# Celebrandil/CudaSift

Hardware: AMD Instinct MI355X
Metric: 1920x1080 SIFT frames/sec (higher is better)
Workload: dtype f32

## Files before the change

### cudasift_amd/csrc/kernels_points.hip

```cpp
#include "common.hpp"

#define WAVES_PER_BLOCK 4

__device__ __forceinline__ void wave_sync()
{
  __builtin_amdgcn_fence(__ATOMIC_RELEASE, "wavefront");
  __builtin_amdgcn_wave_barrier();
  __builtin_amdgcn_fence(__ATOMIC_ACQUIRE, "wavefront");
}

template <int CTRL, int ROW_MASK>
__device__ __forceinline__ float dpp_f(float v)
{
  return __builtin_bit_cast(float, __builtin_amdgcn_update_dpp(0, __builtin_bit_cast(int, v), CTRL, ROW_MASK, 0xf, false));
}
#define DPP_QUAD_XOR1 0xB1
#define DPP_QUAD_XOR2 0x4E
#define DPP_ROW_HALF_MIRROR 0x141
#define DPP_ROW_MIRROR 0x140
#define DPP_ROW_BCAST15 0x142
#define DPP_ROW_BCAST31 0x143

__device__ __forceinline__ float wave_sum(float v)
{
// ... 827 lines not shown
  const int stride = gridDim.x * WAVES_PER_BLOCK;
  const int tr = lane >> 4, tc = lane & 15;
  auto fetch = [&](const float4 &k, const OctaveInfo &L, float (&T)[4]) {
    const float *img = scratch + (long long)frame * P.frame_stride + L.img_off;
    const bool sane = k.x > -64.0f && k.y > -64.0f && k.x < (float)(L.w + 64) && k.y < (float)(L.h + 64);
#if ORIENT_FETCH_CONST
    const int x0 = (sane ? 0 : 1) - 7, y0 = -7;
#else
    const int x0 = (int)floorf(sane ? k.x : 0.0f) - 7, y0 = (int)floorf(sane ? k.y : 0.0f) - 7;
#endif
    const unsigned col = (unsigned)clampi(x0 + tc, 0, L.w - 1);
#pragma unroll
    for (int q = 0; q < 4; q++)
      T[q] = *reinterpret_cast<const float *>(reinterpret_cast<const char *>(img) +
                                              (__umul24((unsigned)clampi(y0 + tr + 4 * q, 0, L.h - 1), (unsigned)L.p) + col) * 4u);
  };
  int idx = __builtin_amdgcn_readfirstlane(blockIdx.x * WAVES_PER_BLOCK + wave);
  int o, i, o1 = 0, i1 = 0, o2 = 0, i2 = 0;
  bool more = flat_to_octave(fc, P.noct, idx, o, i);
  if (!more) return;
  float4 cur = *reinterpret_cast<const float4 *>(&fdet[(size_t)(o - 1) * max_pts + i]), nxt = cur, nxt2 = cur;
  bool more1 = flat_to_octave(fc, P.noct, idx + stride, o1, i1);
  if (more1) nxt = *reinterpret_cast<const float4 *>(&fdet[(size_t)(o1 - 1) * max_pts + i1]);
  float T[4];
  fetch(cur, P.o[o], T);
  while (more) {
    const OctaveInfo &L = P.o[o];
    const float *img = scratch + (long long)frame * P.frame_stride + L.img_off;
    Detection *d = &fdet[(size_t)(o - 1) * max_pts + i];
    const int co = o;
    const bool sane = cur.x > -64.0f && cur.y > -64.0f && cur.x < (float)(L.w + 64) && cur.y < (float)(L.h + 64);
    const int x0 = (int)floorf(sane ? cur.x : 0.0f) - 7, y0 = (int)floorf(sane ? cur.y : 0.0f) - 7;
#pragma unroll
    for (int q = 0; q < 4; q++) s_tile[wave][lane + 64 * q] = T[q];
    wave_sync();
    if (more1) fetch(nxt, P.o[o1], T);
    const bool more2 = more1 && flat_to_octave(fc, P.noct, idx + 2 * stride, o2, i2);
    if (more2) nxt2 = *reinterpret_cast<const float4 *>(&fdet[(size_t)(o2 - 1) * max_pts + i2]);
    const OrientResult r = sane ? orient_core_tile(img, L.w, L.h, L.p, q8, cur.x, cur.y, cur.z, s_tile[wave], x0, y0,
                                                   s_hist[wave], s_gauss[wave], s_smp[wave], s_tgrid[wave], lane)
                                : orient_core(img, L.w, L.h, L.p, q8, cur.x, cur.y, cur.z, s_hist[wave], s_gauss[wave],
                                              s_smp[wave], s_tgrid[wave], lane);
    if (lane == 0) {
      d->ori1 = r.ori1;
      d->ori2 = r.ori2;
      d->dupslot = r.has2 ? (int)atomicAdd(&cnt[CNT_DUP + co], 1u) : -1;
    }
    idx += stride;
    more = more1; o = o1; i = i1; cur = nxt;
    more1 = more2; o1 = o2; i1 = i2; nxt = nxt2;
  }
}

template <bool UNROLL>
__device__ __forceinline__ void descr_samples_tile(const float *tile, int x0, int y0, bool q8, float px, float py,
                                                   float sina, float cosa, float ssina, float scosa,
                                                   const float *gauss, int lane, float (&vx)[4], float (&vy)[4],
                                                   int (&ang)[4])
{
  const int tx = lane & 15;
  const float fx = tx - 7.5f, gx = gauss[tx];
  const float *porg = tile_origin<PW>(tile, x0, y0);
#pragma unroll
  for (int j = 0; j < 4; j++) { vx[j] = 0.0f; vy[j] = 0.0f; ang[j] = 0; }
  if (UNROLL) {
#pragma unroll
    for (int j = 0; j < 4; j++) {
      const int y = (lane >> 4) + 4 * j;
      const float fy = y - 7.5f;
      const float xpos = px + fx * scosa - fy * ssina + 0.5f;
      const float ypos = py + fx * ssina + fy * scosa + 0.5f;
      const float dx = tex2d_tile<PW>(porg, xpos + cosa, ypos + sina, q8) -
                       tex2d_tile<PW>(porg, xpos - cosa, ypos - sina, q8);
      const float dy = tex2d_tile<PW>(porg, xpos - sina, ypos + cosa, q8) -
                       tex2d_tile<PW>(porg, xpos + sina, ypos - cosa, q8);
      const float grad = gauss[y] * gx * sqrtf(dx * dx + dy * dy);
      float angf = 4.0f / 3.1415f * fast_atan2(dy, dx) + 4.0f;
      const int angi = (int)angf;
      angf -= angi;
      vx[j] = (1.0f - angf) * grad; vy[j] = angf * grad; ang[j] = angi;
    }
    return;
  }
#pragma unroll 1
  for (int j = 0; j < 4; j++) {
    const int y = (lane >> 4) + 4 * j;
    const float fy = y - 7.5f;
    const float xpos = px + fx * scosa - fy * ssina + 0.5f;
    const float ypos = py + fx * ssina + fy * scosa + 0.5f;
    const float dx = tex2d_tile<PW>(porg, xpos + cosa, ypos + sina, q8) -
                     tex2d_tile<PW>(porg, xpos - cosa, ypos - sina, q8);
    const float dy = tex2d_tile<PW>(porg, xpos - sina, ypos + cosa, q8) -
                     tex2d_tile<PW>(porg, xpos + sina, ypos - cosa, q8);
    const float grad = gauss[y] * gx * sqrtf(dx * dx + dy * dy);
    float angf = 4.0f / 3.1415f * fast_atan2(dy, dx) + 4.0f;
    const int angi = (int)angf;
    angf -= angi;
    const float tvx = (1.0f - angf) * grad, tvy = angf * grad;
    vx[0] = j == 0 ? tvx : vx[0]; vy[0] = j == 0 ? tvy : vy[0]; ang[0] = j == 0 ? angi : ang[0];
    vx[1] = j == 1 ? tvx : vx[1]; vy[1] = j == 1 ? tvy : vy[1]; ang[1] = j == 1 ? angi : ang[1];
    vx[2] = j == 2 ? tvx : vx[2]; vy[2] = j == 2 ? tvy : vy[2]; ang[2] = j == 2 ? angi : ang[2];
    vx[3] = j == 3 ? tvx : vx[3]; vy[3] = j == 3 ? tvy : vy[3]; ang[3] = j == 3 ? angi : ang[3];
  }
}

__device__ __forceinline__ void footprint_weights_init(float *wt, int lane)
{
  const int my = lane >> 3, mx = lane & 7;
  const float wy = my < 4 ? (my + 0.5f) * 0.25f : (3.5f - (my - 4)) * 0.25f;
  const float wx = mx < 4 ? (mx + 0.5f) * 0.25f : (7.5f - mx) * 0.25f;
  wt[lane] = wy * wx;
}
__device__ __forceinline__ float footprint_sum2(const float *base, const float *wt, float acc)
{
#pragma unroll 1
  for (int h = 0; h < 2; h++) {
#pragma unroll
    for (int r = 0; r < 4; r++) {
      const int my = 4 * h + r;
      const float4 lo = *reinterpret_cast<const float4 *>(base + my * SMP_W);
      const float4 hi = *reinterpret_cast<const float4 *>(base + my * SMP_W + 4);
      const float4 wl = *reinterpret_cast<const float4 *>(wt + 8 * my);
      const float4 wh = *reinterpret_cast<const float4 *>(wt + 8 * my + 4);
      acc = __builtin_fmaf(wl.x, lo.x, acc);
      acc = __builtin_fmaf(wl.y, lo.y, acc);
      acc = __builtin_fmaf(wl.z, lo.z, acc);
      acc = __builtin_fmaf(wl.w, lo.w, acc);
      acc = __builtin_fmaf(wh.x, hi.x, acc);
      acc = __builtin_fmaf(wh.y, hi.y, acc);
      acc = __builtin_fmaf(wh.z, hi.z, acc);
      acc = __builtin_fmaf(wh.w, hi.w, acc);
    }
  }
// ... 108 lines not shown
    const unsigned pos = pos0 + 4 * SMP_W * j;
    sx[j] = ang[j] >= 8 ? (unsigned)dump : __umul24(bx & 3u, SMP_PLANE) + pos;
    sy[j] = __umul24(by & 3u, SMP_PLANE) + pos;
    has8 |= ang[j] >= 8;
  }
#pragma unroll
  for (int j = 0; j < 4; j++) {
    tbl[sx[j]] = ang[j] < 4 ? vx[j] : 0.0f;
    tbl[sy[j]] = (ang[j] < 3 || ang[j] >= 7) ? vy[j] : 0.0f;
  }
  wave_sync();
  float acc0 = FOOTPRINT_SUM(mine, nullptr, 0.0f);
  wave_sync();
#pragma unroll
  for (int j = 0; j < 4; j++) {
    tbl[sx[j]] = ang[j] < 4 ? 0.0f : vx[j];
    tbl[sy[j]] = (ang[j] < 3 || ang[j] >= 7) ? 0.0f : vy[j];
  }
  wave_sync();
  float acc1 = FOOTPRINT_SUM(mine, nullptr, 0.0f);
  wave_sync();
#pragma unroll
  for (int j = 0; j < 4; j++) {
    tbl[sx[j]] = 0.0f;
    tbl[sy[j]] = 0.0f;
  }
  if (__any(has8)) {
    wave_sync();
#pragma unroll
    for (int j = 0; j < 4; j++)
      if (ang[j] >= 8) tbl[pos0 + 4 * SMP_W * j] = vx[j];
    wave_sync();
    if ((lane & 3) == 0 && cell >= 1) {
      const int pc = cell - 1, pcx = pc & 3, pcy = pc >> 2;
      acc0 = FOOTPRINT_SUM(tbl + (4 * pcy) * SMP_W + 4 * pcx, nullptr, acc0);
    }
    wave_sync();
#pragma unroll
    for (int j = 0; j < 4; j++)
      if (ang[j] >= 8) tbl[pos0 + 4 * SMP_W * j] = 0.0f;
  }
  const float tsum1 = wave_sum(acc0 * acc0 + acc1 * acc1);
  const float rs1 = 1.0f / sqrtf(tsum1);
  const float c0 = fminf(acc0 * rs1, 0.2f), c1 = fminf(acc1 * rs1, 0.2f);
  const float tsum2 = wave_sum(c0 * c0 + c1 * c1);
  const float rs2 = 1.0f / sqrtf(tsum2);
  out0 = c0 * rs2;
  out1 = c1 * rs2;
}
#ifndef DESCR_SCATTER_SELECT
#define DESCR_SCATTER_SELECT 1
#endif

__device__ __forceinline__ void descr_write(SiftPointD *sift, SiftPointD *pack_dst, int pack_off, unsigned pack_cnt,
                                            unsigned dst, int lane, float o0, float o1v, const Detection &d,
                                            float orientation, float subsampling, float out_scale)
{
  const int cell = lane >> 2;
#pragma unroll
  for (int tgt = 0; tgt < 2; tgt++) {
    SiftPointD *p = tgt == 0 ? (sift ? &sift[dst] : nullptr)
                             : (pack_dst && dst < pack_cnt ? pack_dst + pack_off + dst : nullptr);
    if (!p) continue;
    p->data[8 * cell + (lane & 3)] = o0;
    p->data[8 * cell + (lane & 3) + 4] = o1v;
    if (lane == 0) {
      p->xpos = d.xpos * subsampling * out_scale;
      p->ypos = d.ypos * subsampling * out_scale;
      p->scale = d.scale * subsampling * out_scale;
      p->sharpness = d.sharpness;
      p->edgeness = d.edgeness;
      p->orientation = orientation;
      p->subsampling = subsampling;
      if (tgt == 1) {
        p->score = 0.0f; p->ambiguity = 0.0f; p->match = 0; p->match_xpos = 0.0f; p->match_ypos = 0.0f;
        p->match_error = 0.0f; p->empty[0] = 0.0f; p->empty[1] = 0.0f; p->empty[2] = 0.0f;
      }
    }
  }
}

#ifndef DESCR_OCC
#define DESCR_OCC 4
#endif
#ifndef DESCR_UNROLL_SAMPLES
#define DESCR_UNROLL_SAMPLES 1
#endif
struct alignas(16) DescrWaveLds {
  float buf[PATCH_FLOATS];
  float park[12 * 64];
  float gauss[16];
  float wtab[64];
};
template <bool Q8, bool BAL, bool FUSE = false>
__device__ __forceinline__ void descr_all_body(const float *__restrict__ scratch, const PyramidInfo &P,
                                               unsigned *__restrict__ counters, const Detection *__restrict__ det,
                                               SiftPointD *__restrict__ pts, int max_pts,
                                               const int *__restrict__ pack_offsets, SiftPointD *__restrict__ pack_dst,
                                               unsigned *__restrict__ big_list, unsigned big_stride, DescrWaveLds *s_w,
                                               const int4 *__restrict__ block_map, const unsigned *fdup = nullptr,
                                               int fuse_items = 0)
{
  static_assert(PATCH_FLOATS == 4 * SMP_PLANE, "the window and the four vote planes share one buffer");
  const int wave = threadIdx.x >> 6, lane = threadIdx.x & 63;
  const FrameShare fs = frame_share<BAL>(block_map);
  if (BAL && fs.frame < 0) return;
  const int frame = fs.frame;
  unsigned *cnt = counters + (size_t)frame * CNT_STRIDE;
  const Detection *fdet = det + (size_t)frame * MISIFT_MAX_OCTAVES * max_pts;
  SiftPointD *sift = pts ? pts + (size_t)frame * max_pts : nullptr;
  const int pack_off = pack_dst ? __builtin_amdgcn_readfirstlane(pack_offsets[frame]) : 0;
  const unsigned pack_cnt = pack_dst ? (unsigned)(__builtin_amdgcn_readfirstlane(pack_offsets[frame + 1]) - pack_off) : 0u;
  const bool q8 = Q8;
  float *buf = s_w[wave].buf;
  const float *gauss = s_w[wave].gauss;
  if (lane < 16) s_w[wave].gauss[lane] = det_exp(-(lane - 7.5f) * (lane - 7.5f) / 128.0f);
  if (!DESCR_FOOT_LITERAL) footprint_weights_init(s_w[wave].wtab, lane);
  if (!FUSE && fs.sub == 0 && threadIdx.x == 0) {
    unsigned b = 0;
    for (int k = 1; k <= P.noct; k++) {
      __hip_atomic_store(&cnt[2 * k - 1], b, __ATOMIC_RELAXED, __HIP_MEMORY_SCOPE_AGENT);
      b += cnt[CNT_DET + k];
      __hip_atomic_store(&cnt[2 * k], b, __ATOMIC_RELAXED, __HIP_MEMORY_SCOPE_AGENT);
      b += cnt[CNT_DUP + k];
      __hip_atomic_store(&cnt[2 * k + 1], b, __ATOMIC_RELAXED, __HIP_MEMORY_SCOPE_AGENT);
    }
  }
  const int stride = FUSE ? 1 : fs.nsub * WAVES_PER_BLOCK;
  auto ndet = [&](int k) -> int {
// ... 80 lines not shown
      for (int k = 0; k < nori; k++) {
        if (k == 1) {
#pragma unroll
          for (int j = 0; j < 4; j++) {
            park[64 * j] = vx[j];
            park[64 * (4 + j)] = vy[j];
            park[64 * (8 + j)] = __builtin_bit_cast(float, ang[j]);
          }
        }
        const float theta = 2.0f * 3.1415f / 360.0f * ((k == 0 && doA) ? d.ori1 : d.ori2);
        float sina, cosa;
        det_sincos(theta, sina, cosa);
        descr_samples_tile<DESCR_UNROLL_SAMPLES>(buf, g.x0, g.y0, q8, d.xpos, d.ypos, sina, cosa, scale * sina, scale * cosa, gauss, lane, vx, vy, ang);
      }
      wave_sync();
      {
        float *z = buf + 4 * lane_i;
#pragma unroll
        for (int k = 0; k < 6; k++) *reinterpret_cast<float4 *>(z + 256 * k) = make_float4(0.0f, 0.0f, 0.0f, 0.0f);
        int lane_k = lane;
        asm volatile("" : "+v"(lane_k));
        buf[1536 + lane_k] = 0.0f;
      }
      wave_sync();
#pragma unroll 1
      for (int k = nori - 1; k >= 0; k--) {
        if (k == 0 && nori == 2) {
#pragma unroll
          for (int j = 0; j < 4; j++) {
            vx[j] = park[64 * j];
            vy[j] = park[64 * (4 + j)];
            ang[j] = __builtin_bit_cast(int, park[64 * (8 + j)]);
          }
        }
        const bool first = k == 0 && doA;
        float o0, o1v;
#if DESCR_SCATTER_SELECT && DESCR_FOOT_LITERAL
        descr_accumulate_sel(buf, (int)((offsetof(DescrWaveLds, wtab) - offsetof(DescrWaveLds, buf)) / sizeof(float)) + lane, lane,
                             vx, vy, ang, o0, o1v);
#else
        descr_accumulate(buf, s_w[wave].wtab, lane, vx, vy, ang, o0, o1v);
#endif
        descr_write(sift, pack_dst, pack_off, pack_cnt, first ? dstA : dstB, lane, o0, o1v, d, first ? d.ori1 : d.ori2,
                    subsampling, (!first && o == P.noct && !P.fix_numpts) ? 1.0f : P.out_scale);
      }
    }
    wave_sync();
    more = more1; o = o1; i = i1; g = g1;
    more1 = more2; o1 = o2; i1 = i2; h1 = h2;
    (void)lim; (void)lim1;
  }
}

template <bool Q8>
__device__ __forceinline__ void descr_big_frame(const float *__restrict__ scratch, const PyramidInfo &P,
                                                const unsigned *__restrict__ cnt, const Detection *__restrict__ det,
                                                SiftPointD *__restrict__ pts, int max_pts,
                                                const int *__restrict__ pack_offsets, SiftPointD *__restrict__ pack_dst,
                                                const unsigned *__restrict__ big_list, unsigned big_stride, unsigned nbig,
                                                float *s_smp_w, float *s_gauss_w, int lane, int frame, unsigned first,
                                                unsigned step)
{
  const Detection *fdet = det + (size_t)frame * MISIFT_MAX_OCTAVES * max_pts;
  SiftPointD *sift = pts ? pts + (size_t)frame * max_pts : nullptr;
  const int pack_off = pack_dst ? pack_offsets[frame] : 0;
  const unsigned pack_cnt = pack_dst ? (unsigned)(pack_offsets[frame + 1] - pack_off) : 0u;
  descr_init(s_smp_w, s_gauss_w, lane);
  for (unsigned t = first; t < nbig; t += step) {
    const unsigned code = big_list[(size_t)frame * big_stride + t];
    const int o = (int)(code >> 24), i = (int)(code & 0xffffffu);
    const OctaveInfo &L = P.o[o];
    const float *img = scratch + (long long)frame * P.frame_stride + L.img_off;
    const Detection d = fdet[(size_t)(o - 1) * max_pts + i];
    unsigned b = 0;
    for (int k = 1; k < o; k++) b += cnt[CNT_DET + k] + cnt[CNT_DUP + k];
    const unsigned bdet = b, bdup = b + cnt[CNT_DET + o];
    for (int which = 0; which < 2; which++) {
      if (which == 1 && d.dupslot < 0) break;
      const unsigned dst = which == 0 ? bdet + (unsigned)i : bdup + (unsigned)d.dupslot;
      if (dst >= (unsigned)max_pts) continue;
      float o0, o1v;
      descr_core(img, L.w, L.h, L.p, Q8, d.xpos, d.ypos, d.scale, which == 0 ? d.ori1 : d.ori2, s_smp_w, s_gauss_w,
                 lane, o0, o1v);
      descr_write(sift, pack_dst, pack_off, pack_cnt, dst, lane, o0, o1v, d, which == 0 ? d.ori1 : d.ori2, L.subsampling,
                  (which == 1 && o == P.noct && !P.fix_numpts) ? 1.0f : P.out_scale);
    }
  }
}

__device__ __forceinline__ void export_counters_host(const unsigned *counters, unsigned nframes, unsigned *host_out,
                                                     unsigned host_seq)
{
  const unsigned nwords = nframes * CNT_STRIDE;
  for (unsigned w = threadIdx.x; w < nwords; w += blockDim.x)
    host_out[w] = __hip_atomic_load(counters + w, __ATOMIC_RELAXED, __HIP_MEMORY_SCOPE_SYSTEM);
  __threadfence_system();
  __syncthreads();
  if (threadIdx.x == 0) __hip_atomic_store(host_out + nwords, host_seq, __ATOMIC_RELEASE, __HIP_MEMORY_SCOPE_SYSTEM);
}
__device__ __forceinline__ bool last_workgroup(unsigned *counters)
{
  __shared__ unsigned s_last;
  asm volatile("s_waitcnt vmcnt(0)" ::: "memory");
  __builtin_amdgcn_fence(__ATOMIC_RELEASE, "workgroup");
  __syncthreads();
  if (threadIdx.x == 0) s_last = atomicAdd(counters + CNT_TICKET, 1u) == gridDim.x * gridDim.y - 1 ? 1u : 0u;
  __syncthreads();
  return s_last != 0;
}

__device__ __forceinline__ bool last_workgroup_2level(unsigned *spare)
{
  __shared__ unsigned s_last2;
  asm volatile("s_waitcnt vmcnt(0)" ::: "memory");
  __builtin_amdgcn_fence(__ATOMIC_RELEASE, "workgroup");
  __syncthreads();
  if (threadIdx.x == 0) {
    const unsigned nwg = gridDim.x * gridDim.y, lb = blockIdx.y * gridDim.x + blockIdx.x;
    const unsigned sub = lb & 15u, members = (nwg - sub + 15u) / 16u;
    unsigned last = 0u;
    if (atomicAdd(&spare[80 + 32 * sub], 1u) == members - 1u) {
      const unsigned nsub = nwg < 16u ? nwg : 16u;
      if (atomicAdd(&spare[48], 1u) == nsub - 1u) last = 1u;
    }
    s_last2 = last;
  }
  __syncthreads();
  return s_last2 != 0;
}

template <bool Q8, int OCC, bool BAL>
__global__ __launch_bounds__(256, OCC) void descr_all_kernel(const float *__restrict__ scratch, PyramidInfo P,
                                                        unsigned *__restrict__ counters,
                                                        const Detection *__restrict__ det,
                                                        SiftPointD *__restrict__ pts, int max_pts, int frac8,
                                                        const int *__restrict__ pack_offsets,
                                                        SiftPointD *__restrict__ pack_dst,
                                                        unsigned *__restrict__ big_list, unsigned big_stride,
                                                        const int4 *__restrict__ block_map,
                                                        unsigned *__restrict__ tail_host_out, unsigned tail_seq)
{
  __shared__ DescrWaveLds s_w[WAVES_PER_BLOCK];
  descr_all_body<Q8, BAL>(scratch, P, counters, det, pts, max_pts, pack_offsets, pack_dst, big_list, big_stride, s_w,
                          block_map);
  if (!BAL && tail_host_out) {
    if (last_workgroup_2level(counters + (size_t)P.nframes * CNT_STRIDE))
      export_counters_host(counters, (unsigned)P.nframes, tail_host_out, tail_seq);
  }
}

template <bool Q8>
__global__ __launch_bounds__(256) void descr_big_kernel(const float *__restrict__ scratch, PyramidInfo P,
                                                        const unsigned *__restrict__ counters,
                                                        const Detection *__restrict__ det,
                                                        SiftPointD *__restrict__ pts, int max_pts,
                                                        const int *__restrict__ pack_offsets,
                                                        SiftPointD *__restrict__ pack_dst,
                                                        const unsigned *__restrict__ big_list, unsigned big_stride,
                                                        unsigned *__restrict__ host_out, unsigned host_seq)
{
  __shared__ __attribute__((aligned(16))) float s_smp[WAVES_PER_BLOCK][DESCR_TBL];
  __shared__ float s_gauss[WAVES_PER_BLOCK][16];
  const int wave = threadIdx.x >> 6, lane = threadIdx.x & 63;
  const int frame = blockIdx.y;
  const unsigned *cnt = counters + (size_t)frame * CNT_STRIDE;
  const unsigned nbig = min(cnt[CNT_BIG], big_stride);
  if (nbig != 0)
    descr_big_frame<Q8>(scratch, P, cnt, det, pts, max_pts, pack_offsets, pack_dst, big_list, big_stride, nbig,
                        s_smp[wave], s_gauss[wave], lane, frame, blockIdx.x * WAVES_PER_BLOCK + wave,
                        gridDim.x * WAVES_PER_BLOCK);
  if (!host_out) return;
  if (!last_workgroup(const_cast<unsigned *>(counters))) return;
  export_counters_host(counters, gridDim.y, host_out, host_seq);
}

template <bool Q8, bool BAL, bool FUSE = false>
__device__ __forceinline__ void orient_gather_body(const float *__restrict__ scratch, const PyramidInfo &P,
                                                   unsigned *__restrict__ counters, Detection *__restrict__ det, int max_pts,
                                                   const int4 *__restrict__ block_map, float *hist, float *gauss, float2 *smp,
                                                   float *tgrid, unsigned *s_done = nullptr, int fuse_items = 0)
{
  const int wave = threadIdx.x >> 6, lane = threadIdx.x & 63;
  const FrameShare fs = frame_share<BAL>(block_map);
  if (BAL && fs.frame < 0) return;
  const int frame = fs.frame;
  unsigned *cnt = counters + (size_t)frame * CNT_STRIDE;
  Detection *fdet = det + (size_t)frame * MISIFT_MAX_OCTAVES * max_pts;
  const bool q8 = Q8;
  if (lane >= 57) smp[64 + lane] = make_float2(-1.0f, 0.0f);
  const FrameCounts fc = load_frame_counts(cnt, P.noct, max_pts, false);
  const int stride = FUSE ? 1 : fs.nsub * WAVES_PER_BLOCK;
  int idx = __builtin_amdgcn_readfirstlane(fs.sub * WAVES_PER_BLOCK + wave) * (FUSE ? fuse_items : 1);
  const int end = idx + fuse_items;
  int o, i;
  bool more = flat_to_octave(fc, P.noct, idx, o, i);
  float4 nxt = more ? *reinterpret_cast<const float4 *>(&fdet[(size_t)(o - 1) * max_pts + i]) : make_float4(0, 0, 0, 0);
// ... 310 lines not shown
      float4 *dst = reinterpret_cast<float4 *>(&T[lo + rank]);
#pragma unroll 4
      for (int q = 0; q < (int)(sizeof(SiftPointD) / 16); q++) dst[q] = src[q];
    }
  }
}
__global__ __launch_bounds__(256) void sort_copy_back_kernel(SiftPointD *__restrict__ pts, const SiftPointD *__restrict__ tmp,
                                                             const unsigned *__restrict__ counters, int max_pts, int last_slot)
{
  const int frame = blockIdx.y;
  const unsigned *cnt = counters + (size_t)frame * CNT_STRIDE;
  const size_t n = (size_t)min(cnt[last_slot], (unsigned)max_pts) * (sizeof(SiftPointD) / 16);
  float4 *dst = reinterpret_cast<float4 *>(pts + (size_t)frame * max_pts);
  const float4 *src = reinterpret_cast<const float4 *>(tmp + (size_t)frame * max_pts);
  for (size_t q = (size_t)blockIdx.x * 256 + threadIdx.x; q < n; q += (size_t)gridDim.x * 256) dst[q] = src[q];
}

static inline int points_grid_x(misift_ctx *ctx, int nframes, int blocks_per_cu = 0)
{
  if (blocks_per_cu <= 0) blocks_per_cu = ctx->point_blocks_per_cu;
  int per_frame = (ctx->num_cus * blocks_per_cu + nframes - 1) / nframes;
  if (per_frame < 8) per_frame = 8;
  const int cap = nframes <= ctx->small_frames ? 1024 : 512;
  if (per_frame > cap) per_frame = cap;
  return per_frame;
}

#define LAUNCH_Q8(kernel, grid, block, ...)                                                       \
  do {                                                                                            \
    if (ctx->opt.texfrac_bits == 8) hipLaunchKernelGGL(kernel<true>, grid, block, 0, ctx->stream, __VA_ARGS__);   \
    else hipLaunchKernelGGL(kernel<false>, grid, block, 0, ctx->stream, __VA_ARGS__);             \
  } while (0)

int launch_orient(misift_ctx *ctx, const float *base, long long base_frame_stride, int w, int h, int pitch,
                  int nframes, int octave, SiftPointD *pts, int max_pts)
{
  LaunchScope ls(ctx, "orient");
  LAUNCH_Q8(orient_kernel, dim3(points_grid_x(ctx, nframes), nframes), dim3(256), base, base_frame_stride, w, h, pitch,
            octave, ctx->d_counters, pts, max_pts, 0);
  return ls.finish();
}

int launch_descr(misift_ctx *ctx, const float *base, long long base_frame_stride, int w, int h, int pitch,
                 int nframes, float subsampling, int octave, SiftPointD *pts, int max_pts)
{
  LaunchScope ls(ctx, "descr");
  LAUNCH_Q8(descr_kernel, dim3(points_grid_x(ctx, nframes), nframes), dim3(256), base, base_frame_stride, w, h, pitch,
            subsampling, octave, ctx->d_counters, pts, max_pts, 0);
  return ls.finish();
}

static int prepare_block_maps(misift_ctx *ctx, const PyramidInfo &P, bool *wanted);

int launch_bin_detections(misift_ctx *ctx, const PyramidInfo &P, int max_pts)
{
  bool balanced = false;
  int rc = prepare_block_maps(ctx, P, &balanced);
  if (rc) return rc;
  FrameSharesArgs sh = {0, 0, nullptr, nullptr};
  if (balanced) {
    sh.t_a = ctx->map_t_orient; sh.t_b = ctx->map_t_descr;
    sh.map_a = ctx->d_block_map; sh.map_b = ctx->d_block_map + ctx->map_t_orient;
  }
  LaunchScope ls(ctx, "bin_detections");
  hipLaunchKernelGGL(bin_detections_kernel, dim3(P.noct + (balanced ? 1 : 0), P.nframes), dim3(256), 0, ctx->stream, P,
                     ctx->d_counters, ctx->d_det, ctx->d_det_sorted, max_pts, ctx->opt.deterministic ? 1 : 0, sh);
  rc = ls.finish();
  if (rc == MISIFT_OK && balanced) ctx->cur_balanced = 1;
  return rc;
}

int launch_renumber_dups(misift_ctx *ctx, const PyramidInfo &P, int max_pts)
{
  LaunchScope ls(ctx, "renumber_dups");
  hipLaunchKernelGGL(renumber_dups_kernel, dim3(P.noct, P.nframes), dim3(256), 0, ctx->stream, P, ctx->d_counters,
                     ctx->d_det_sorted, max_pts);
  return ls.finish();
}

static int prepare_block_maps(misift_ctx *ctx, const PyramidInfo &P, bool *wanted)
{
  *wanted = false;
  if (!ctx->balance_frames || P.nframes <= ctx->small_frames || ctx->in_capture || ctx->tile_orient || !ctx->tile_descr)
    return MISIFT_OK;
  const int t_orient = points_grid_x(ctx, P.nframes, ctx->orient_blocks_per_cu) * P.nframes;
  const int t_descr = points_grid_x(ctx, P.nframes) * P.nframes;
  if (ctx->block_map_cap < t_orient + t_descr) {
    if (ctx->d_block_map) HIP_TRY(misift_dev_free(ctx->d_block_map));
    ctx->d_block_map = nullptr; ctx->block_map_cap = 0;
    HIP_TRY(misift_dev_alloc((void **)&ctx->d_block_map, sizeof(int4) * (size_t)(t_orient + t_descr), "block_maps"));
    ctx->block_map_cap = t_orient + t_descr;
    ctx->alloc_gen++;
  }
  ctx->map_t_orient = t_orient; ctx->map_t_descr = t_descr;
  *wanted = true;
  return MISIFT_OK;
}

static int build_block_maps(misift_ctx *ctx, const PyramidInfo &P, int max_pts)
{
  if (ctx->cur_balanced) return MISIFT_OK;
  bool wanted = false;
  int rc = prepare_block_maps(ctx, P, &wanted);
  if (rc || !wanted) return rc;
  LaunchScope ls(ctx, "frame_shares");
  hipLaunchKernelGGL(frame_shares_kernel, dim3(1), dim3(256), 0, ctx->stream, ctx->d_counters, P.nframes, P.noct, max_pts,
                     ctx->map_t_orient, ctx->d_block_map, ctx->map_t_descr, ctx->d_block_map + ctx->map_t_orient);
  rc = ls.finish();
  if (rc == MISIFT_OK) ctx->cur_balanced = 1;
  return rc;
}

int launch_orient_all(misift_ctx *ctx, const float *scratch, const PyramidInfo &P, SiftPointD *pts, int max_pts)
{
  (void)pts;
  {
    int rc = build_block_maps(ctx, P, max_pts);
    if (rc) return rc;
  }
  LaunchScope ls(ctx, "orient_all");
  Detection *det = ctx->cur_binned ? ctx->d_det_sorted : ctx->d_det;
  const dim3 grid(points_grid_x(ctx, P.nframes, ctx->orient_blocks_per_cu), P.nframes);
  const bool q8 = ctx->opt.texfrac_bits == 8;
  if (ctx->tile_orient) LAUNCH_Q8(orient_all_kernel, grid, dim3(256), scratch, P, ctx->d_counters, det, max_pts, 0);
  else if (ctx->cur_balanced) {
    const dim3 flat(ctx->map_t_orient);
    if (q8) hipLaunchKernelGGL((orient_all_gather_kernel<true, true>), flat, dim3(256), (size_t)ctx->lds_pad_orient, ctx->stream, scratch, P,
                               ctx->d_counters, det, max_pts, 0, ctx->d_block_map);
    else hipLaunchKernelGGL((orient_all_gather_kernel<false, true>), flat, dim3(256), (size_t)ctx->lds_pad_orient, ctx->stream, scratch, P,
                            ctx->d_counters, det, max_pts, 0, ctx->d_block_map);
  } else {
    if (q8) hipLaunchKernelGGL((orient_all_gather_kernel<true, false>), grid, dim3(256), (size_t)ctx->lds_pad_orient, ctx->stream, scratch, P,
                               ctx->d_counters, det, max_pts, 0, (const int4 *)nullptr);
    else hipLaunchKernelGGL((orient_all_gather_kernel<false, false>), grid, dim3(256), (size_t)ctx->lds_pad_orient, ctx->stream, scratch, P,
                            ctx->d_counters, det, max_pts, 0, (const int4 *)nullptr);
  }
  return ls.finish();
}

int launch_descr_all(misift_ctx *ctx, const float *scratch, const PyramidInfo &P, SiftPointD *pts, int max_pts,
                     const int *pack_offsets, SiftPointD *pack_dst)
{
  LaunchScope ls(ctx, "descr_all");
  const Detection *det = ctx->cur_binned ? ctx->d_det_sorted : ctx->d_det;
  const dim3 grid(points_grid_x(ctx, P.nframes), P.nframes);
  if (ctx->tile_descr) {
    unsigned big_stride = 0;
    for (int o = 1; o <= P.noct; o++) big_stride += P.o[o].cand_cap;
    unsigned *host_out = nullptr;
    if (ctx->want_export && !ctx->in_capture) {
      host_out = ctx->h_counters;
      ctx->export_seq++;
      ctx->exported = 1;
    }
    const bool bal = ctx->cur_balanced != 0;
    const bool fold = host_out && !bal && ctx->fold_descr_tail && P.nframes <= ctx->small_frames;
    const dim3 dgrid = bal ? dim3(ctx->map_t_descr) : grid;
    const int4 *bmap = bal ? ctx->d_block_map + ctx->map_t_orient : nullptr;
    unsigned *tail_out = fold ? host_out : nullptr;
#define DESCR_LAUNCH(Q, O, B) hipLaunchKernelGGL((descr_all_kernel<Q, O, B>), dgrid, dim3(256), (size_t)ctx->lds_pad_descr, ctx->stream, scratch, P, \
                                                 ctx->d_counters, det, pts, max_pts, 0, pack_offsets, pack_dst, ctx->d_cand, \
                                                 big_stride, bmap, tail_out, ctx->export_seq)
#define DESCR_LAUNCH_B(Q, O) do { if (bal) DESCR_LAUNCH(Q, O, true); else DESCR_LAUNCH(Q, O, false); } while (0)
    const bool q8 = ctx->opt.texfrac_bits == 8;
    if (ctx->descr_occ >= 4) { if (q8) DESCR_LAUNCH_B(true, 4); else DESCR_LAUNCH_B(false, 4); }
    else { if (q8) DESCR_LAUNCH_B(true, 3); else DESCR_LAUNCH_B(false, 3); }
#undef DESCR_LAUNCH_B
#undef DESCR_LAUNCH
    PendingBig &pb = ctx->pending_big;
    pb.valid = 0;
    if (fold) {
      pb.valid = 1; pb.scratch = scratch; pb.P = P; pb.det = det; pb.pts = pts; pb.max_pts = max_pts;
      pb.pack_offsets = pack_offsets; pb.pack_dst = pack_dst; pb.big_stride = big_stride;
    } else {
      LAUNCH_Q8(descr_big_kernel, dim3(2, P.nframes), dim3(256), scratch, P, ctx->d_counters, det, pts, max_pts,
                pack_offsets, pack_dst, ctx->d_cand, big_stride, host_out, ctx->export_seq);
    }
  } else
    LAUNCH_Q8(descr_all_gather_kernel, grid, dim3(256), scratch, P, ctx->d_counters, det, pts, max_pts, 0, pack_offsets,
              pack_dst);
  return ls.finish();
}

int launch_orient_descr_fused(misift_ctx *ctx, const float *scratch, const PyramidInfo &P, SiftPointD *pts, int max_pts)
{
  LaunchScope ls(ctx, "orient_descr");
  Detection *det = ctx->d_det;
  const dim3 grid(points_grid_x(ctx, P.nframes), P.nframes);
  unsigned big_stride = 0;
  for (int o = 1; o <= P.noct; o++) big_stride += P.o[o].cand_cap;
  unsigned *host_out = nullptr;
  if (ctx->want_export && !ctx->in_capture) {
    host_out = ctx->h_counters;
    ctx->export_seq++;
    ctx->exported = 1;
  }
  const bool fold = host_out && ctx->fold_descr_tail;
  unsigned *tail_out = fold ? host_out : nullptr;
  const bool q8 = ctx->opt.texfrac_bits == 8;
#define FUSED_LAUNCH(Q, O) hipLaunchKernelGGL((orient_descr_fused_kernel<Q, O>), grid, dim3(256), (size_t)ctx->lds_pad_descr, ctx->stream, \
                                              scratch, P, ctx->d_counters, det, pts, max_pts, ctx->d_cand, big_stride,                \
                                              ctx->fuse_wait_ticks, tail_out, ctx->export_seq)
  if (!q8) FUSED_LAUNCH(false, 3);
  else if (ctx->descr_occ >= 4) FUSED_LAUNCH(true, 4);
  else FUSED_LAUNCH(true, 3);
#undef FUSED_LAUNCH
  PendingBig &pb = ctx->pending_big;
  pb.valid = 0;
  if (fold) {
    pb.valid = 1; pb.scratch = scratch; pb.P = P; pb.det = det; pb.pts = pts; pb.max_pts = max_pts;
    pb.pack_offsets = nullptr; pb.pack_dst = nullptr; pb.big_stride = big_stride;
  } else {
    LAUNCH_Q8(descr_big_kernel, dim3(2, P.nframes), dim3(256), scratch, P, ctx->d_counters, det, pts, max_pts,
              (const int *)nullptr, (SiftPointD *)nullptr, ctx->d_cand, big_stride, host_out, ctx->export_seq);
  }
  return ls.finish();
}

int launch_descr_big_pending(misift_ctx *ctx)
// ... 65 lines not shown
```

Measured before the change: 58120.

## Add smaller-LDS descriptor kernel with direct global-to-LDS window loads for higher occupancy

Adds a new descriptor kernel variant whose per-wave LDS footprint drops the park area and shares the patch buffer with the vote planes, so six workgroups can fit per CU. Interior patch windows are loaded with global_load_lds DMA instead of going through registers, and a half-unrolled sampling loop plus opaque uniform values are used to hold down register pressure. The grid size is scaled to match the higher occupancy. The path only runs when descr_occ is set to 5 or higher, and it brings extra sync points and reuses one buffer, which carries some correctness risk.

```diff
diff --git a/cudasift_amd/csrc/kernels_points.hip b/cudasift_amd/csrc/kernels_points.hip
--- a/cudasift_amd/csrc/kernels_points.hip
+++ b/cudasift_amd/csrc/kernels_points.hip
@@ -903,7 +903,7 @@
   }
 }
 
-template <bool UNROLL>
+template <int UNROLL>
 __device__ __forceinline__ void descr_samples_tile(const float *tile, int x0, int y0, bool q8, float px, float py,
                                                    float sina, float cosa, float ssina, float scosa,
                                                    const float *gauss, int lane, float (&vx)[4], float (&vy)[4],
@@ -914,7 +914,7 @@
   const float *porg = tile_origin<PW>(tile, x0, y0);
 #pragma unroll
   for (int j = 0; j < 4; j++) { vx[j] = 0.0f; vy[j] = 0.0f; ang[j] = 0; }
-  if (UNROLL) {
+  if (UNROLL == 1) {
 #pragma unroll
     for (int j = 0; j < 4; j++) {
       const int y = (lane >> 4) + 4 * j;
@@ -930,6 +930,34 @@
       const int angi = (int)angf;
       angf -= angi;
       vx[j] = (1.0f - angf) * grad; vy[j] = angf * grad; ang[j] = angi;
+    }
+    return;
+  }
+  if (UNROLL == 2) {
+#pragma unroll 1
+    for (int jj = 0; jj < 2; jj++) {
+      float tvx[2], tvy[2];
+      int tan[2];
+#pragma unroll
+      for (int u = 0; u < 2; u++) {
+        const int y = (lane >> 4) + 4 * (2 * jj + u);
+        const float fy = y - 7.5f;
+        const float xpos = px + fx * scosa - fy * ssina + 0.5f;
+        const float ypos = py + fx * ssina + fy * scosa + 0.5f;
+        const float dx = tex2d_tile<PW>(porg, xpos + cosa, ypos + sina, q8) -
+                         tex2d_tile<PW>(porg, xpos - cosa, ypos - sina, q8);
+        const float dy = tex2d_tile<PW>(porg, xpos - sina, ypos + cosa, q8) -
+                         tex2d_tile<PW>(porg, xpos + sina, ypos - cosa, q8);
+        const float grad = gauss[y] * gx * sqrtf(dx * dx + dy * dy);
+        float angf = 4.0f / 3.1415f * fast_atan2(dy, dx) + 4.0f;
+        const int angi = (int)angf;
+        angf -= angi;
+        tvx[u] = (1.0f - angf) * grad; tvy[u] = angf * grad; tan[u] = angi;
+      }
+      vx[0] = jj == 0 ? tvx[0] : vx[0]; vy[0] = jj == 0 ? tvy[0] : vy[0]; ang[0] = jj == 0 ? tan[0] : ang[0];
+      vx[1] = jj == 0 ? tvx[1] : vx[1]; vy[1] = jj == 0 ? tvy[1] : vy[1]; ang[1] = jj == 0 ? tan[1] : ang[1];
+      vx[2] = jj == 1 ? tvx[0] : vx[2]; vy[2] = jj == 1 ? tvy[0] : vy[2]; ang[2] = jj == 1 ? tan[0] : ang[2];
+      vx[3] = jj == 1 ? tvx[1] : vx[3]; vy[3] = jj == 1 ? tvy[1] : vy[3]; ang[3] = jj == 1 ? tan[1] : ang[3];
     }
     return;
   }
@@ -1144,9 +1172,16 @@
 #define DESCR_SCATTER_SELECT 1
 #endif
 
+__device__ __forceinline__ float opaque_uniform(float x)
+{
+  int v = __builtin_amdgcn_readfirstlane(__builtin_bit_cast(int, x));
+  asm volatile("" : "+s"(v));
+  return __builtin_bit_cast(float, v);
+}
+template <bool ZERO_ARG = false>
 __device__ __forceinline__ void descr_write(SiftPointD *sift, SiftPointD *pack_dst, int pack_off, unsigned pack_cnt,
                                             unsigned dst, int lane, float o0, float o1v, const Detection &d,
-                                            float orientation, float subsampling, float out_scale)
+                                            float orientation, float subsampling, float out_scale, float zero = 0.0f)
 {
   const int cell = lane >> 2;
 #pragma unroll
@@ -1165,8 +1200,13 @@
       p->orientation = orientation;
       p->subsampling = subsampling;
       if (tgt == 1) {
-        p->score = 0.0f; p->ambiguity = 0.0f; p->match = 0; p->match_xpos = 0.0f; p->match_ypos = 0.0f;
-        p->match_error = 0.0f; p->empty[0] = 0.0f; p->empty[1] = 0.0f; p->empty[2] = 0.0f;
+        if (ZERO_ARG) {
+          p->score = zero; p->ambiguity = zero; p->match = __builtin_bit_cast(int, zero); p->match_xpos = zero; p->match_ypos = zero;
+          p->match_error = zero; p->empty[0] = zero; p->empty[1] = zero; p->empty[2] = zero;
+        } else {
+          p->score = 0.0f; p->ambiguity = 0.0f; p->match = 0; p->match_xpos = 0.0f; p->match_ypos = 0.0f;
+          p->match_error = 0.0f; p->empty[0] = 0.0f; p->empty[1] = 0.0f; p->empty[2] = 0.0f;
+        }
       }
     }
   }
@@ -1353,6 +1393,192 @@
   }
 }
 
+struct alignas(16) DescrWinLds {
+  float buf[PATCH_FLOATS];
+  float gauss[16];
+#if DESCR_SCATTER_SELECT && DESCR_FOOT_LITERAL
+  float dump[16];
+#else
+  float wtab[64];
+#endif
+};
+#if DESCR_SCATTER_SELECT && DESCR_FOOT_LITERAL
+static_assert(sizeof(DescrWinLds) == 6528, "6 workgroups of 4 wavefronts per CU within 160 KB");
+#endif
+#define WIN_PIECES 7
+__device__ __forceinline__ void window_dma(const float *img, int pitch, const PatchGeom &g, int lane, float *buf)
+{
+  static_assert(PW == 40 && PATCH_FLOATS * 4 == 6 * 1024 + 16 * 16, "six whole pieces, then lanes 0..15 of a seventh");
+  typedef const __attribute__((address_space(1))) void *gptr_t;
+  typedef __attribute__((address_space(3))) void *lptr_t;
+  unsigned lo[5];
+#pragma unroll
+  for (int j = 0; j < 5; j++) {
+    const unsigned t = (unsigned)lane + 64u * j;
+    const unsigned r = __umul24(t, 6554u) >> 16;
+    const unsigned c4 = (t - __umul24(r, 10u)) * 4u;
+    lo[j] = (__umul24(r, (unsigned)pitch) + c4) * 4u;
+  }
+#pragma unroll
+  for (int k = 0; k < WIN_PIECES; k++) {
+    const int j = k % 5, m = k / 5;
+    const char *base = reinterpret_cast<const char *>(img + (size_t)(g.y0 + 32 * m) * pitch + g.x0);
+    if (k < WIN_PIECES - 1 || lane < 16)
+      __builtin_amdgcn_global_load_lds((gptr_t)(base + lo[j]), (lptr_t)(buf + 256 * k), 16, 0, 0);
+  }
+}
+
+template <bool Q8, bool BAL, int UNROLL>
+__device__ __forceinline__ void descr_win_body(const float *__restrict__ scratch, const PyramidInfo &P,
+                                               unsigned *__restrict__ counters, const Detection *__restrict__ det,
+                                               SiftPointD *__restrict__ pts, int max_pts,
+                                               const int *__restrict__ pack_offsets, SiftPointD *__restrict__ pack_dst,
+                                               unsigned *__restrict__ big_list, unsigned big_stride, DescrWinLds *s_w,
+                                               const int4 *__restrict__ block_map)
+{
+  static_assert(PATCH_FLOATS == 4 * SMP_PLANE, "the window and the four vote planes share one buffer");
+  const int wave = threadIdx.x >> 6, lane = threadIdx.x & 63;
+  const FrameShare fs = frame_share<BAL>(block_map);
+  if (BAL && fs.frame < 0) return;
+  const int frame = fs.frame;
+  unsigned *cnt = counters + (size_t)frame * CNT_STRIDE;
+  const Detection *fdet = det + (size_t)frame * MISIFT_MAX_OCTAVES * max_pts;
+  SiftPointD *sift = pts ? pts + (size_t)frame * max_pts : nullptr;
+  const int pack_off = pack_dst ? __builtin_amdgcn_readfirstlane(pack_offsets[frame]) : 0;
+  const unsigned pack_cnt = pack_dst ? (unsigned)(__builtin_amdgcn_readfirstlane(pack_offsets[frame + 1]) - pack_off) : 0u;
+  const bool q8 = Q8;
+  float *buf = s_w[wave].buf;
+  const float *gauss = s_w[wave].gauss;
+  if (lane < 16) s_w[wave].gauss[lane] = det_exp(-(lane - 7.5f) * (lane - 7.5f) / 128.0f);
+#if !(DESCR_SCATTER_SELECT && DESCR_FOOT_LITERAL)
+  footprint_weights_init(s_w[wave].wtab, lane);
+#endif
+  if (fs.sub == 0 && threadIdx.x == 0) {
+    unsigned b = 0;
+    for (int k = 1; k <= P.noct; k++) {
+      __hip_atomic_store(&cnt[2 * k - 1], b, __ATOMIC_RELAXED, __HIP_MEMORY_SCOPE_AGENT);
+      b += cnt[CNT_DET + k];
+      __hip_atomic_store(&cnt[2 * k], b, __ATOMIC_RELAXED, __HIP_MEMORY_SCOPE_AGENT);
+      b += cnt[CNT_DUP + k];
+      __hip_atomic_store(&cnt[2 * k + 1], b, __ATOMIC_RELAXED, __HIP_MEMORY_SCOPE_AGENT);
+    }
+  }
+  const int stride = fs.nsub * WAVES_PER_BLOCK;
+  auto ndet = [&](int k) -> int {
+    return (int)min(__builtin_amdgcn_readfirstlane(cnt[CNT_DET + k]), (unsigned)max_pts);
+  };
+  auto advance = [&](int &o, int &i, int &lim, int by) -> bool {
+    i += by;
+    while (i >= lim) {
+      i -= lim;
+      o++;
+      if (o > P.noct) return false;
+      lim = ndet(o);
+    }
+    return true;
+  };
+  auto head = [&](int oo, int ii) -> float4 {
+    const Detection &r = fdet[(size_t)(oo - 1) * max_pts + ii];
+    return make_float4(r.xpos, r.ypos, r.scale, 0.0f);
+  };
+  int o = 1, i = 0, lim = ndet(1);
+  bool more = advance(o, i, lim, __builtin_amdgcn_readfirstlane(fs.sub * WAVES_PER_BLOCK + wave));
+  if (!more) return;
+  int o1 = o, i1 = i, lim1 = lim;
+  bool more1 = advance(o1, i1, lim1, stride);
+  float4 h1 = head(o, i);
+  PatchGeom g = patch_geom(h1.x, h1.y, h1.z, P.o[o].w, P.o[o].h, P.patch_reach);
+  if (more1) h1 = head(o1, i1);
+  int cur_o = 0;
+  unsigned bdet = 0, bdup = 0;
+  while (more) {
+    const OctaveInfo &L = P.o[o];
+    const float subsampling = L.subsampling;
+    const Detection d = fdet[(size_t)(o - 1) * max_pts + i];
+    if (o != cur_o) {
+      unsigned b = 0;
+      for (int k = 1; k < o; k++)
+        b += __builtin_amdgcn_readfirstlane(cnt[CNT_DET + k]) + __builtin_amdgcn_readfirstlane(cnt[CNT_DUP + k]);
+      bdet = b;
+      bdup = b + __builtin_amdgcn_readfirstlane(cnt[CNT_DET + o]);
+      cur_o = o;
+    }
+    const unsigned dstA = bdet + (unsigned)i;
+    const bool dup = d.dupslot >= 0;
+    const unsigned dstB = bdup + (unsigned)(dup ? d.dupslot : 0);
+    const bool doA = dstA < (unsigned)max_pts, doB = dup && dstB < (unsigned)max_pts;
+    if (!g.fits) {
+      if (lane == 0 && (doA || doB)) {
+        const unsigned slot = atomicAdd(&cnt[CNT_BIG], 1u);
+        if (slot < big_stride)
+          big_list[(size_t)frame * big_stride + slot] = ((unsigned)o << 24) | (unsigned)i;
+      }
+    } else if (doA || doB) {
+      const float *img = scratch + (long long)frame * P.frame_stride + L.img_off;
+      const bool interior = g.x0 >= 0 && g.y0 >= 0 && g.x0 + PW <= L.w && g.y0 + PW <= L.h;
+      const float scale = 12.0f / 16.0f * d.scale;
+      const int nori = (doA ? 1 : 0) + (doB ? 1 : 0);
+#pragma unroll 1
+      for (int k = 0; k < nori; k++) {
+        const bool first = k == 0 && doA;
+        int lane_i = lane;
+        asm volatile("" : "+v"(lane_i));
+        asm volatile("s_waitcnt lgkmcnt(0)" ::: "memory");
+        if (interior) window_dma(img, L.p, g, lane_i, buf);
+        else {
+          float R[PATCH_LOADS];
+          patch_fetch(img, L.w, L.h, L.p, g, lane_i, R);
+          patch_store(buf, lane_i, R);
+        }
+        const float theta = 2.0f * 3.1415f / 360.0f * (first ? d.ori1 : d.ori2);
+        float sina, cosa;
+        det_sincos(theta, sina, cosa);
+        asm volatile("s_waitcnt vmcnt(0)" ::: "memory");
+        wave_sync();
+        float vx[4], vy[4];
+        int ang[4];
+        int lane_s = lane;
+        asm volatile("" : "+v"(lane_s));
+        descr_samples_tile<UNROLL>(buf, g.x0, g.y0, q8, d.xpos, d.ypos, sina, cosa, scale * sina, scale * cosa, gauss, lane_s, vx, vy, ang);
+        wave_sync();
+        {
+          float *z = buf + 4 * lane_i;
+#pragma unroll
+          for (int q = 0; q < 6; q++) *reinterpret_cast<float4 *>(z + 256 * q) = make_float4(0.0f, 0.0f, 0.0f, 0.0f);
+          int lane_k = lane;
+          asm volatile("" : "+v"(lane_k));
+          buf[1536 + lane_k] = 0.0f;
+        }
+        wave_sync();
+        float o0, o1v;
+        int lane_a = lane;
+        asm volatile("" : "+v"(lane_a));
+#if DESCR_SCATTER_SELECT && DESCR_FOOT_LITERAL
+        descr_accumulate_sel(buf, (int)((offsetof(DescrWinLds, dump) - offsetof(DescrWinLds, buf)) / sizeof(float)) + (lane_a & 15),
+                             lane_a, vx, vy, ang, o0, o1v);
+#else
+        descr_accumulate(buf, s_w[wave].wtab, lane_a, vx, vy, ang, o0, o1v);
+#endif
+        Detection dw = d;
+        float ori = first ? d.ori1 : d.ori2, sub = subsampling;
+        dw.xpos = opaque_uniform(dw.xpos); dw.ypos = opaque_uniform(dw.ypos); dw.scale = opaque_uniform(dw.scale);
+        dw.sharpness = opaque_uniform(dw.sharpness); dw.edgeness = opaque_uniform(dw.edgeness);
+        ori = opaque_uniform(ori); sub = opaque_uniform(sub);
+        int lane_w = lane;
+        asm volatile("" : "+v"(lane_w));
+        descr_write<true>(sift, pack_dst, pack_off, pack_cnt, first ? dstA : dstB, lane_w, o0, o1v, dw, ori, sub,
+                    (!first && o == P.noct && !P.fix_numpts) ? 1.0f : P.out_scale, opaque_uniform(0.0f));
+        wave_sync();
+      }
+    }
+    more = more1; o = o1; i = i1;
+    if (more) g = patch_geom(h1.x, h1.y, h1.z, P.o[o].w, P.o[o].h, P.patch_reach);
+    more1 = more && advance(o1, i1, lim1, stride);
+    if (more1) h1 = head(o1, i1);
+    (void)lim;
+  }
+}
+
 template <bool Q8>
 __device__ __forceinline__ void descr_big_frame(const float *__restrict__ scratch, const PyramidInfo &P,
                                                 const unsigned *__restrict__ cnt, const Detection *__restrict__ det,
@@ -1443,6 +1669,26 @@
 {
   __shared__ DescrWaveLds s_w[WAVES_PER_BLOCK];
   descr_all_body<Q8, BAL>(scratch, P, counters, det, pts, max_pts, pack_offsets, pack_dst, big_list, big_stride, s_w,
+                          block_map);
+  if (!BAL && tail_host_out) {
+    if (last_workgroup_2level(counters + (size_t)P.nframes * CNT_STRIDE))
+      export_counters_host(counters, (unsigned)P.nframes, tail_host_out, tail_seq);
+  }
+}
+
+template <bool Q8, int OCC, bool BAL>
+__global__ __launch_bounds__(256, OCC) void descr_win_kernel(const float *__restrict__ scratch, PyramidInfo P,
+                                                        unsigned *__restrict__ counters,
+                                                        const Detection *__restrict__ det,
+                                                        SiftPointD *__restrict__ pts, int max_pts, int frac8,
+                                                        const int *__restrict__ pack_offsets,
+                                                        SiftPointD *__restrict__ pack_dst,
+                                                        unsigned *__restrict__ big_list, unsigned big_stride,
+                                                        const int4 *__restrict__ block_map,
+                                                        unsigned *__restrict__ tail_host_out, unsigned tail_seq)
+{
+  __shared__ DescrWinLds s_w[WAVES_PER_BLOCK];
+  descr_win_body<Q8, BAL, (OCC >= 6 ? (Q8 ? 2 : 0) : 1)>(scratch, P, counters, det, pts, max_pts, pack_offsets, pack_dst, big_list, big_stride, s_w,
                           block_map);
   if (!BAL && tail_host_out) {
     if (last_workgroup_2level(counters + (size_t)P.nframes * CNT_STRIDE))
@@ -1859,6 +2105,15 @@
 
 static int prepare_block_maps(misift_ctx *ctx, const PyramidInfo &P, bool *wanted);
 
+static inline int descr_win_occ(const misift_ctx *ctx) { return ctx->descr_occ >= 6 ? 6 : ctx->descr_occ == 5 ? 5 : 0; }
+static inline int descr_blocks_per_cu(const misift_ctx *ctx)
+{
+  const int occ = descr_win_occ(ctx);
+  if (!occ || !ctx->tile_descr) return ctx->point_blocks_per_cu;
+  const int b = ctx->point_blocks_per_cu * occ / 4;
+  return b > 0 ? b : 1;
+}
+
 int launch_bin_detections(misift_ctx *ctx, const PyramidInfo &P, int max_pts)
 {
   bool balanced = false;
@@ -1891,7 +2146,7 @@
   if (!ctx->balance_frames || P.nframes <= ctx->small_frames || ctx->in_capture || ctx->tile_orient || !ctx->tile_descr)
     return MISIFT_OK;
   const int t_orient = points_grid_x(ctx, P.nframes, ctx->orient_blocks_per_cu) * P.nframes;
-  const int t_descr = points_grid_x(ctx, P.nframes) * P.nframes;
+  const int t_descr = points_grid_x(ctx, P.nframes, descr_blocks_per_cu(ctx)) * P.nframes;
   if (ctx->block_map_cap < t_orient + t_descr) {
     if (ctx->d_block_map) HIP_TRY(misift_dev_free(ctx->d_block_map));
     ctx->d_block_map = nullptr; ctx->block_map_cap = 0;
@@ -1950,7 +2205,7 @@
 {
   LaunchScope ls(ctx, "descr_all");
   const Detection *det = ctx->cur_binned ? ctx->d_det_sorted : ctx->d_det;
-  const dim3 grid(points_grid_x(ctx, P.nframes), P.nframes);
+  const dim3 grid(points_grid_x(ctx, P.nframes, descr_blocks_per_cu(ctx)), P.nframes);
   if (ctx->tile_descr) {
     unsigned big_stride = 0;
     for (int o = 1; o <= P.noct; o++) big_stride += P.o[o].cand_cap;
@@ -1970,8 +2225,16 @@
                                                  big_stride, bmap, tail_out, ctx->export_seq)
 #define DESCR_LAUNCH_B(Q, O) do { if (bal) DESCR_LAUNCH(Q, O, true); else DESCR_LAUNCH(Q, O, false); } while (0)
     const bool q8 = ctx->opt.texfrac_bits == 8;
-    if (ctx->descr_occ >= 4) { if (q8) DESCR_LAUNCH_B(true, 4); else DESCR_LAUNCH_B(false, 4); }
+#define DESCR_WIN_LAUNCH(Q, O, B) hipLaunchKernelGGL((descr_win_kernel<Q, O, B>), dgrid, dim3(256), (size_t)ctx->lds_pad_descr, ctx->stream, scratch, P, \
+                                                     ctx->d_counters, det, pts, max_pts, 0, pack_offsets, pack_dst, ctx->d_cand, \
+                                                     big_stride, bmap, tail_out, ctx->export_seq)
+#define DESCR_WIN_LAUNCH_B(Q, O) do { if (bal) DESCR_WIN_LAUNCH(Q, O, true); else DESCR_WIN_LAUNCH(Q, O, false); } while (0)
+    if (descr_win_occ(ctx) == 6) { if (q8) DESCR_WIN_LAUNCH_B(true, 6); else DESCR_WIN_LAUNCH_B(false, 6); }
+    else if (descr_win_occ(ctx) == 5) { if (q8) DESCR_WIN_LAUNCH_B(true, 5); else DESCR_WIN_LAUNCH_B(false, 5); }
+    else if (ctx->descr_occ >= 4) { if (q8) DESCR_LAUNCH_B(true, 4); else DESCR_LAUNCH_B(false, 4); }
     else { if (q8) DESCR_LAUNCH_B(true, 3); else DESCR_LAUNCH_B(false, 3); }
+#undef DESCR_WIN_LAUNCH_B
+#undef DESCR_WIN_LAUNCH
 #undef DESCR_LAUNCH_B
 #undef DESCR_LAUNCH
     PendingBig &pb = ctx->pending_big;
```

New measurement: 57040. 1.9% lower.
